# epam/Zstandard

Measured on AMD Instinct MI355X. Metric: GiB/s compress @ level 3, 64 KiB chunks, higher is better.
Workload: dtype u8; 1 GPU; 4096 independent 65536 B chunks per GPU per step, level 3, BASELINE config[1] shape (Silesia unavailable offline -> Zipf-token log stream, SURVEY 8d); chunks_per_gpu=4096, chunk_bytes=65536, level=3, parallelism=chunks sharded over 1 GPU(s), no collective in the data path

## Files before the change

zstandard_amd/csrc/lz_kernels.hip:

```cpp
#include "zsmi_device.h"
#include <type_traits>

#ifndef ZS_CAND_G
#define ZS_CAND_G 8
#endif
#ifndef ZS_CAND_G_BIG
#define ZS_CAND_G_BIG 16
#endif
#define ZS_CAND_GOF(TLOG) ((TLOG) > ZS_TABLE_LOG_SMALL ? ZS_CAND_G_BIG : ZS_CAND_G)
#ifndef ZS_CAND_DEPTH
#define ZS_CAND_DEPTH 2
#endif
#ifndef ZS_CAND_RUNS
#define ZS_CAND_RUNS 1
#endif
#define ZS_CAND_WAVES(NT) (3 * (NT))
#define ZS_CAND_ROW 65u
#define ZS_CAND_LDS(TLOG, NT) ((size_t)(NT) * (4u << (TLOG)) + 3u * (NT) * ZS_CAND_GOF(TLOG) * ZS_CAND_ROW * 4u + (NT) * 256u + 3u * 16u * 8u + 32u)
#define ZS_SLOT_EMPTY 0xFFFFFFFFu
__device__ __forceinline__ uint32_t zs_hash_short(uint32_t lo, uint32_t hi) { return __umul24(lo, 0x9E3779u) + __umul24(__builtin_amdgcn_alignbit(hi, lo, 16), 0x85EBCBu); }
__device__ __forceinline__ uint32_t zs_hash_long(uint32_t lo, uint32_t hi)
{ return __umul24(lo, 0x9E3779u) + __umul24(__builtin_amdgcn_alignbit(hi, lo, 24), 0x85EBCBu) + __umul24(hi >> 16, 0xC2B2AFu); }

template <int TLOG, int NT, bool PFX = false>
__global__ void __launch_bounds__(64 * ZS_CAND_WAVES(NT))
k_lz_candidates(const uint8_t *__restrict__ src, const ZsUnitDesc *__restrict__ units, uint32_t block0,
                uint16_t *__restrict__ distAll, uint8_t *__restrict__ distHiAll, uint32_t *__restrict__ candCount,
                const uint32_t *__restrict__ dictImg = nullptr, uint32_t pfx = 0)
{
    static_assert(!PFX || TLOG == ZS_TABLE_LOG_BIG, "a prefixed unit spans up to 128 KiB of positions");
    extern __shared__ __attribute__((aligned(16))) uint32_t candLds[];
    constexpr bool BIG = TLOG > ZS_TABLE_LOG_SMALL;
    constexpr uint32_t G = ZS_CAND_GOF(TLOG), GP = G * 64u, H = G / NT;
    constexpr uint32_t M = ZS_CAND_DEPTH;
    constexpr uint32_t LPS = 64u / G;
    constexpr uint32_t WD = G / 4u + 2u;
    static_assert(G == 8 || G == 16, "a hasher lane takes G consecutive positions of a group: 8 or 16");
    const uint32_t wave = (uint32_t)__builtin_amdgcn_readfirstlane((int)(threadIdx.x >> 6)), lane = threadIdx.x & 63u;
    const uint32_t tab = (wave < NT) ? wave : ((wave < 2 * NT) ? wave - NT : wave - 2 * NT);
    uint32_t *T = candLds + ((size_t)tab << TLOG);
    uint32_t *opnd = candLds + ((size_t)NT << TLOG);
    constexpr uint32_t ROW = ZS_CAND_ROW, GR = G * ROW;
    constexpr uint32_t RING = 3u * NT * GR;
    uint64_t *runMarks = reinterpret_cast<uint64_t *>(opnd + RING + NT * 64u);
    uint32_t *runFlag = opnd + RING + NT * 64u + 3u * 16u * 2u;
    const ZsUnitDesc ud = units[blockIdx.x];
    const uint8_t *s = src + ud.srcOff;
    const uint32_t n = ud.size;
    const size_t slot = (size_t)(ud.firstBlock - block0);
    uint16_t *dist = distAll + slot * ZS_BLOCK_MAX;
    uint8_t *distHi = distHiAll + slot * (ZS_BLOCK_MAX / 8);
    const uint32_t hashable = (n >= 8) ? n - 7 : 0;
    const uint32_t nGroups = (hashable + GP - 1) / GP;
    if (threadIdx.x < 2) candCount[2 * slot + threadIdx.x] = 0;
    if (nGroups == 0) return;
    if (n >= 16 && (n & 15u) == 0) {
        uint4 f;
        __builtin_memcpy(&f, s, 16);
        const uint32_t splat = (f.x & 0xFFu) * 0x01010101u;
        if (((f.x ^ splat) | (f.y ^ splat) | (f.z ^ splat) | (f.w ^ splat)) == 0) {
            if (threadIdx.x == 0) candLds[0] = 0;
            __syncthreads();
            uint32_t mixed = 0;
            for (uint32_t i = threadIdx.x * 16u; i < n && !mixed; i += ZS_CAND_WAVES(NT) * 64u * 16u) {
                uint4 v;
                __builtin_memcpy(&v, s + i, 16);
                mixed = (v.x ^ splat) | (v.y ^ splat) | (v.z ^ splat) | (v.w ^ splat);
            }
            if (mixed) candLds[0] = 1u;
            __syncthreads();
            const bool uniform = candLds[0] == 0;
            __syncthreads();
            if (uniform) return;
        }
    }
    const uint32_t dummyBase = ((uint32_t)(NT - tab) << TLOG) + RING + tab * 64u;
    auto mergeRead = [&](uint32_t g, uint32_t (&mS)[H], uint32_t (&mL)[H]) {
        const uint32_t *xb = opnd + (size_t)(g % 3u) * NT * GR + (NT > 1 ? tab * H : 0u) * ROW + lane;
        #pragma unroll
        for (uint32_t uu = 0; uu < H; uu++) { mS[uu] = xb[uu * ROW]; mL[uu] = (NT > 1) ? xb[GR + uu * ROW] : 0u; }
    };
    uint32_t found = 0;
    const uint32_t matchlessBelow = n >> ZS_MATCHLESS_SHIFT;
    auto mergeStore = [&](uint32_t g, const uint32_t (&mS)[H], const uint32_t (&mL)[H]) {
        const uint32_t sbase = g * GP + ((NT > 1) ? tab * H * 64u : 0u);
        uint64_t hiMine = 0;
        #pragma unroll
        for (uint32_t uu = 0; uu < H; uu++) {
            const uint32_t dm = (NT > 1) ? (mL[uu] ? mL[uu] : mS[uu]) : mS[uu];
            if (BIG) { const uint64_t hi = __ballot((dm >> 16) != 0); if (lane == uu) hiMine = hi; }
            if (found < matchlessBelow) {
                if ((g + 1u) * GP <= hashable) found += (uint32_t)__popcll(__ballot(dm != 0));
                else found += (uint32_t)__popcll(__ballot(dm != 0 && sbase + uu * 64 + lane < hashable));
            }
            dist[sbase + uu * 64 + lane] = (uint16_t)dm;
        }
        if (BIG && lane < H) *reinterpret_cast<uint64_t *>(distHi + ((sbase + lane * 64) >> 3)) = hiMine;
    };
    if (wave >= 2 * NT) {
        __syncthreads(); __syncthreads();
        for (uint32_t i = 2; i <= nGroups + 1; i++) {
            uint32_t mS[H], mL[H];
            mergeRead(i - 2, mS, mL);
#if ZS_CAND_RUNS
            if (__builtin_amdgcn_readfirstlane((int)runFlag[((i - 2) % 3u) * 2u + tab])) {
                if (lane == 0) runFlag[((i - 2) % 3u) * 2u + tab] = 0;
                #pragma unroll
                for (uint32_t uu = 0; uu < H; uu++) {
                    const uint64_t marks = runMarks[((i - 2) % 3u) * 16u + ((NT > 1) ? tab * H : 0u) + uu];
                    if ((marks >> lane) & 1ull) { if (NT > 1) mL[uu] = 1u; else mS[uu] = 1u; }
                }
            }
#endif
            mergeStore(i - 2, mS, mL);
            __syncthreads();
        }
        if (lane == 0) candCount[2 * slot + tab] = found;
        return;
    }

    if (wave < NT) {
        if constexpr (PFX) {
            uint4 *t4 = reinterpret_cast<uint4 *>(T);
            const uint4 *img4 = reinterpret_cast<const uint4 *>(dictImg + ((size_t)tab << TLOG));
            #pragma unroll 8
            for (uint32_t i = lane; i < (1u << TLOG) / 4; i += 64) t4[i] = img4[i];
        } else {
            uint4 *t4 = reinterpret_cast<uint4 *>(T);
            const uint4 e = make_uint4(ZS_SLOT_EMPTY, ZS_SLOT_EMPTY, ZS_SLOT_EMPTY, ZS_SLOT_EMPTY);
            #pragma unroll 8
            for (uint32_t i = lane; i < (1u << TLOG) / 4; i += 64) t4[i] = e;
        }
        uint32_t ringSlot = 0;
        __syncthreads();
        for (uint32_t i = 1; i <= nGroups; i++) {
            uint32_t *ob = opnd + ((size_t)ringSlot * NT + tab) * GR + lane;
            const uint32_t base = (i - 1) * GP + lane + (PFX ? pfx : 0u);
            uint32_t op[G], entry[G], old[G];
            #pragma unroll
            for (uint32_t u = 0; u < G; u++) op[u] = ob[u * ROW];
            #pragma unroll
            for (uint32_t u = 0; u < G; u++) {
                uint32_t pu = base + u * 64u;
                asm volatile("" : "+v"(pu));
                entry[u] = (op[u] & 0xFFFE0000u) | pu;
                old[u] = atomicExch(&T[op[u] & 0xFFFFu], entry[u]);
            }
            #pragma unroll
            for (uint32_t u = 0; u < G; u++) {
                const uint32_t x = old[u] ^ entry[u], dd = entry[u] - old[u];
                ob[u * ROW] = (max(x, dd) < (1u << 17)) ? dd : 0u;
            }
            ringSlot = (ringSlot == 2u) ? 0u : ringSlot + 1u;
            __syncthreads();
        }
        __syncthreads();
        return;
    }

    auto run = [&](auto roleTag) {
        constexpr bool LONG = decltype(roleTag)::value;
        const uint32_t stepOfLane = lane / LPS, l0 = (lane % LPS) * G;
        const uint32_t wbase = stepOfLane * ROW + l0;
        const uint32_t last8 = n - 8;
        auto loadGroup = [&](uint32_t g, uint32_t (&w)[WD]) {
            const uint32_t o = g * GP + lane * G;
            #pragma unroll
            for (uint32_t k = 0; k < WD / 2; k++) {
                const uint32_t ok = o + 8u * k, oc = min(ok, last8);
                const uint64_t v = zs_load64(s + oc) >> (8u * min(ok - oc, 7u));
                w[2 * k] = (uint32_t)v; w[2 * k + 1] = (uint32_t)(v >> 32);
            }
        };
        uint32_t bufA[M][WD], bufB[M][WD];
        auto loadM = [&](uint32_t g0, uint32_t (&buf)[M][WD]) {
            #pragma unroll
            for (uint32_t k = 0; k < M; k++) loadGroup(min(g0 + k, nGroups), buf[k]);
        };
        auto iter = [&](auto wholeTag, uint32_t i, const uint32_t (&w)[WD]) {
            constexpr bool WHOLE = decltype(wholeTag)::value;
            const uint32_t ringSlot = i % 3u;
            if (i < nGroups) {
                uint32_t *ob = opnd + ((size_t)ringSlot * NT + tab) * GR + wbase;
                const uint32_t pbase = i * GP + lane * G;
                #pragma unroll
                for (uint32_t u = 0; u < G; u++) {
                    const uint32_t k = u >> 2, sh = u & 3u;
                    const uint32_t lo = sh ? __builtin_amdgcn_alignbyte(w[k + 1], w[k], sh) : w[k];
                    const uint32_t hi = sh ? __builtin_amdgcn_alignbyte(w[min(k + 2, WD - 1)], w[k + 1], sh) : w[k + 1];
                    uint32_t h = LONG ? zs_hash_long(lo, hi) : zs_hash_short(lo, hi);
                    asm volatile("" : "+v"(h));
                    const uint32_t r = __builtin_amdgcn_alignbit(h, h, 32 - TLOG);
                    ob[u] = (WHOLE || pbase + u < hashable) ? (r & (0xFFFE0000u | ((1u << TLOG) - 1u))) : ((r & 0xFFFE0000u) | (dummyBase + l0 + u));
                }
#if ZS_CAND_RUNS
                bool flat = false;
                uint64_t flatLanes = 0;
                if (WHOLE && __ballot(w[0] == w[1])) {
                    uint32_t diff = w[0] ^ __builtin_amdgcn_alignbyte(w[0], w[0], 1);
                    #pragma unroll
                    for (uint32_t k = 1; k < WD; k++) diff |= w[k] ^ w[k - 1];
                    flat = diff == 0;
                    flatLanes = __ballot(flat);
                }
                if (flatLanes) {
                    const uint32_t key = flat ? ((w[0] & 0xFFu) | 0x100u) : 0u;
                    const uint32_t keyBelow = (uint32_t)__builtin_amdgcn_update_dpp(0, (int)key, 0x138, 0xF, 0xF, true);
                    const uint32_t keyAbove = (uint32_t)__builtin_amdgcn_update_dpp(0, (int)key, 0x130, 0xF, 0xF, true);
                    const bool markFirst = flat && keyBelow == key && (lane % LPS) != 0u;
                    const bool innerLast = flat && keyAbove == key && (lane % LPS) != LPS - 1u;
                    if (flat) {
                        uint32_t h = LONG ? zs_hash_long(w[0], w[1]) : zs_hash_short(w[0], w[1]);
                        asm volatile("" : "+v"(h));
                        const uint32_t away = (__builtin_amdgcn_alignbit(h, h, 32 - TLOG) & 0xFFFE0000u) | (dummyBase + l0);
                        if (markFirst) ob[0] = away;
                        #pragma unroll
                        for (uint32_t u = 1; u + 1 < G; u++) ob[u] = away + u;
                        if (innerLast) ob[G - 1] = away + (G - 1);
                    }
                    if (!LONG) {
                        if (lane < NT) runFlag[ringSlot * 2u + lane] = 1u;
                        const uint32_t bits = flat ? (((1u << G) - 2u) | (markFirst ? 1u : 0u)) : 0u;
                        if (G == 8) reinterpret_cast<uint8_t *>(runMarks + ringSlot * 16u)[lane] = (uint8_t)bits;
                        else reinterpret_cast<uint16_t *>(runMarks + ringSlot * 16u)[lane] = (uint16_t)bits;
                    }
                }
#endif
            }
            __syncthreads();
        };
        auto step = [&](uint32_t i, const uint32_t (&w)[WD]) {
            if (i > nGroups + 1) return;
            if ((i + 1) * GP + 8u <= n) iter(std::true_type{}, i, w); else iter(std::false_type{}, i, w);
        };
#if ZS_CAND_RUNS
        if (!LONG && lane < 6u) runFlag[lane] = 0;
#endif
        loadM(0, bufA);
        for (uint32_t g0 = 0; g0 <= nGroups + 1; g0 += 2 * M) {
            loadM(g0 + M, bufB);
            #pragma unroll
            for (uint32_t k = 0; k < M; k++) step(g0 + k, bufA[k]);
            loadM(g0 + 2 * M, bufA);
            #pragma unroll
            for (uint32_t k = 0; k < M; k++) step(g0 + M + k, bufB[k]);
        }
    };
    if (tab == 0) run(std::false_type{}); else run(std::true_type{});
}

__global__ void __launch_bounds__(1024)
k_lz_dict_tables(const uint8_t *__restrict__ pre, uint32_t pfx, uint32_t *__restrict__ img)
{
    constexpr int TLOG = ZS_TABLE_LOG_BIG;
    __shared__ uint32_t T[1u << TLOG];
    const uint32_t tab = blockIdx.x, tid = threadIdx.x;
    for (uint32_t i = tid; i < (1u << TLOG); i += 1024) T[i] = 0;
    __syncthreads();
    const uint32_t hashable = pfx >= 8 ? pfx - 7 : 0;
    for (uint32_t p = tid; p < hashable; p += 1024) {
        const uint64_t v = zs_load64(pre + p);
        const uint32_t lo = (uint32_t)v, hi = (uint32_t)(v >> 32);
        const uint32_t h = tab ? zs_hash_long(lo, hi) : zs_hash_short(lo, hi);
        const uint32_t r = __builtin_amdgcn_alignbit(h, h, 32 - TLOG);
        atomicMax(&T[r & ((1u << TLOG) - 1u)], ((p + 1u) << 15) | (r >> 17));
    }
    __syncthreads();
    uint32_t *out = img + ((size_t)tab << TLOG);
    for (uint32_t i = tid; i < (1u << TLOG); i += 1024) {
        const uint32_t k = T[i];
        out[i] = k ? (((k & 0x7FFFu) << 17) | ((k >> 15) - 1u)) : ZS_SLOT_EMPTY;
    }
}

#ifndef ZS_WALK_MASK
#define ZS_WALK_MASK 2
#endif
#ifndef ZS_WALK_MINW
#define ZS_WALK_MINW 1
#endif
#define ZS_WALK_WGRP(WLOG) ((WLOG) >= 9 ? 4 : 2)
#ifndef ZS_WALK_LPW_256
#define ZS_WALK_LPW_256 2
#endif
#ifndef ZS_WALK_LPW_512
#define ZS_WALK_LPW_512 4
#endif
#define ZS_WALK_LPW(WLOG) ((WLOG) >= 9 ? ZS_WALK_LPW_512 : ZS_WALK_LPW_256)
#define ZS_WALK_THREADS(BIG, WLOG) ((((BIG) ? ZS_UNIT_MAX : ZS_BLOCK_MAX) >> (WLOG)) * ZS_WALK_LPW(WLOG))
#define ZS_WALK_KERNEL(LOOK, REPW, BIG, WLOG) k_lz_walk<ZS_WALK_LPW(WLOG), ZS_WALK_WGRP(WLOG), LOOK, REPW, BIG, ZS_WALK_THREADS(BIG, WLOG)>
#ifndef ZS_WALK_SKEW
#define ZS_WALK_SKEW  24u
#endif
#define ZS_WALK_FRONT 48u
#define ZS_WALK_TAIL  144u
#define ZS_WALK_SRCBYTES(CAPB) ((((CAPB) + ZS_WALK_TAIL + ZS_WALK_SKEW * (((CAPB) + ZS_WALK_TAIL) / 256u + 1u)) + 15u) & ~15u)
#define ZS_WALK_LDS(CAPB) ((CAPB) / 8 + 16 + ZS_WALK_FRONT + ZS_WALK_SRCBYTES(CAPB) + 16 + 1024)

typedef const __attribute__((address_space(3))) uint32_t *ZsLdsU32;
template <int K>
__device__ __forceinline__ void lds_span(uint32_t byteOff, uint32_t (&out)[K])
{
    ZsLdsU32 d = (ZsLdsU32)(uintptr_t)(byteOff & ~3u);
    uint32_t w[K + 1];
    #pragma unroll
    for (int k = 0; k <= K; k++) w[k] = d[k];
    const uint32_t sh = byteOff & 3u;
    #pragma unroll
    for (int k = 0; k < K; k++) out[k] = __builtin_amdgcn_alignbyte(w[k + 1], w[k], sh);
}
template <int I, int K>
__device__ __forceinline__ uint32_t span_at(const uint32_t (&v)[K])
{
    if constexpr ((I & 3) == 0) return v[I >> 2];
    else return __builtin_amdgcn_alignbyte(v[(I >> 2) + 1], v[I >> 2], I & 3);
}
__device__ __forceinline__ uint32_t zs_agree16(const uint32_t (&a)[4], const uint32_t (&b)[4])
{
    const uint64_t x0 = (uint64_t)(a[0] ^ b[0]) | ((uint64_t)(a[1] ^ b[1]) << 32), x1 = (uint64_t)(a[2] ^ b[2]) | ((uint64_t)(a[3] ^ b[3]) << 32);
    const uint32_t n0 = x0 ? ((uint32_t)__builtin_ctzll(x0) >> 3) : 8u;
    const uint32_t n1 = x1 ? ((uint32_t)__builtin_ctzll(x1) >> 3) : 8u;
    return (n0 < 8u) ? n0 : 8u + n1;
}
template <int LPW> __device__ __forceinline__ uint32_t walker_or(uint32_t v)
{
    if constexpr (LPW >= 2) v |= (uint32_t)__builtin_amdgcn_update_dpp(0, (int)v, 0xB1, 0xF, 0xF, false);
    if constexpr (LPW == 4) v |= (uint32_t)__builtin_amdgcn_update_dpp(0, (int)v, 0x4E, 0xF, 0xF, false);
    return v;
}
template <int LPW> __device__ __forceinline__ int walker_max(int v)
{
    if constexpr (LPW >= 2) v = max(v, __builtin_amdgcn_update_dpp(0, v, 0xB1, 0xF, 0xF, false));
    if constexpr (LPW == 4) v = max(v, __builtin_amdgcn_update_dpp(0, v, 0x4E, 0xF, 0xF, false));
    return v;
}
template <int LPW> __device__ __forceinline__ uint32_t walker_min(uint32_t v)
{
    if constexpr (LPW >= 2) v = min(v, (uint32_t)__builtin_amdgcn_update_dpp(0, (int)v, 0xB1, 0xF, 0xF, false));
    if constexpr (LPW == 4) v = min(v, (uint32_t)__builtin_amdgcn_update_dpp(0, (int)v, 0x4E, 0xF, 0xF, false));
    return v;
}
template <int NT, int DIR>
__device__ __forceinline__ uint32_t block_scan_max(uint32_t v, uint32_t *wv, uint32_t tid, uint32_t *total)
{
    const uint32_t lane = tid & 63u, wave = tid >> 6;
    #pragma unroll
    for (int d = 1; d < 64; d <<= 1) {
        const uint32_t o = (uint32_t)(DIR > 0 ? __shfl_up((int)v, d) : __shfl_down((int)v, d));
        if (DIR > 0 ? (int)lane >= d : (int)lane + d < 64) v = max(v, o);
    }
    __syncthreads();
    if (lane == (DIR > 0 ? 63u : 0u)) wv[wave] = v;
    __syncthreads();
    uint32_t pre = 0, all = 0;
    #pragma unroll
    for (uint32_t k = 0; k < NT / 64; k++) { const uint32_t x = wv[k]; all = max(all, x); if (DIR > 0 ? k < wave : k > wave) pre = max(pre, x); }
    *total = all;
    return max(v, pre);
}
__device__ __forceinline__ uint32_t zs_nonzero8(const uint4 d)
{
    typedef uint16_t u16x2 __attribute__((ext_vector_type(2)));
    const u16x2 one = { 1, 1 };
    (void)one;
    auto nz = [&](uint32_t w) { uint32_t r; asm("v_pk_min_u16 %0, %1, %2" : "=v"(r) : "v"(w), "v"(0x00010001u)); return r; };
    const uint32_t v = nz(d.x) | (nz(d.y) << 2) | (nz(d.z) << 4) | (nz(d.w) << 6);
    return (v | (v >> 15)) & 0xFFu;
}

#ifdef ZS_WALK_PROFILE
#define WPROF_STAMP(k) { __builtin_amdgcn_sched_barrier(0); unsigned long long t_; asm volatile("s_waitcnt vmcnt(0) lgkmcnt(0)\n\ts_memtime %0\n\ts_waitcnt lgkmcnt(0)" : "=s"(t_) :: "memory"); __builtin_amdgcn_sched_barrier(0); wprof[k] += t_ - wlast; wlast = t_; }
#else
#define WPROF_STAMP(k)
#endif
#define ZS_WALK_KERNEL_PFX(LOOK, REPW, WLOG) k_lz_walk<ZS_WALK_LPW(WLOG), ZS_WALK_WGRP(WLOG), LOOK, REPW, true, ZS_WALK_THREADS(false, WLOG), true>
template <int LPW, int WGRP, int LOOK, int REPWIN, bool BIG, int NT, bool PFX = false>
__global__ void __launch_bounds__(NT, BIG ? 1 : ZS_WALK_MINW)
k_lz_walk(const uint8_t *__restrict__ src, const ZsUnitDesc *__restrict__ units, uint32_t block0,
          const uint16_t *__restrict__ distAll, const uint8_t *__restrict__ distHiAll,
          uint2 *__restrict__ recAll, uint32_t junkSlot, uint4 *__restrict__ resAll, int rangeLogArg, const uint32_t *__restrict__ candCount,
          const uint8_t *__restrict__ pre = nullptr, uint32_t pfx = 0)
{
    static_assert(!PFX || BIG, "a prefixed unit is staged in the 128 KiB layout");
    constexpr uint32_t CAP = BIG ? ZS_UNIT_MAX : ZS_BLOCK_MAX;
    constexpr uint32_t CPL = LOOK / LPW, RPL = REPWIN / LPW, GPL = WGRP / LPW;
    static_assert((LPW == 1 || LPW == 2 || LPW == 4) && WGRP % LPW == 0 && LOOK % LPW == 0 && REPWIN % LPW == 0 && CPL >= 1 && RPL >= 1 && LOOK <= 8 && REPWIN <= 8, "a walker's lanes share the groups and candidates evenly");
    static_assert(NT >= 64 && NT % 64 == 0 && NT * GPL * 16 <= CAP / 8, "the exchange buffer holds 16 bytes a lane and group");
    extern __shared__ __attribute__((aligned(16))) uint8_t walkLds[];
    constexpr uint32_t SRC = CAP / 8 + 16 + ZS_WALK_FRONT;
    auto lposv = [](uint32_t v) { return SRC + v + (uint32_t)__mul24((int)v >> 8, (int)ZS_WALK_SKEW); };
    const uint32_t vb = PFX ? pfx : 0u;
    auto lpos = [&](uint32_t p) { return lposv(p + vb); };
    auto stage16 = [&](uint32_t i, const uint4 v) {
        uint8_t *d = walkLds + lposv(i);
        *reinterpret_cast<uint2 *>(d) = make_uint2(v.x, v.y); *reinterpret_cast<uint2 *>(d + 8) = make_uint2(v.z, v.w);
        const uint32_t o = i & 255u;
        if (o == 0) { *reinterpret_cast<uint2 *>(d - ZS_WALK_SKEW) = make_uint2(v.x, v.y); *reinterpret_cast<uint2 *>(d - ZS_WALK_SKEW + 8) = make_uint2(v.z, v.w); }
        else if (o == 16) *reinterpret_cast<uint2 *>(d - ZS_WALK_SKEW) = make_uint2(v.x, v.y);
    };
    const uint32_t tid = threadIdx.x, lane = tid & 63u;
    const uint32_t rangeLog = (uint32_t)rangeLogArg, R = 1u << rangeLog;
    const ZsUnitDesc ud = units[blockIdx.x];
    const uint32_t slot = ud.firstBlock - block0;
    const uint8_t *s = src + ud.srcOff;
    const uint32_t n = ud.size;
    const uint16_t *dist = distAll + (size_t)slot * ZS_BLOCK_MAX;
    const uint8_t *distHi = distHiAll + (size_t)slot * (ZS_BLOCK_MAX / 8);
    uint4 *xbuf = reinterpret_cast<uint4 *>(walkLds);
    const uint32_t xw = (tid & ~63u) * GPL;
    const uint32_t safeAddr = (xw + lane) * 16u;
    uint32_t *queue = reinterpret_cast<uint32_t *>(walkLds + SRC + ZS_WALK_SRCBYTES(CAP));
    uint4 *res = resAll + (size_t)slot * ZS_RES_PER_BLOCK;
    uint8_t *xhi = reinterpret_cast<uint8_t *>(queue + 4);
    uint2 *recs = recAll + (size_t)slot * (ZS_BLOCK_MAX / 4);
    const uint32_t sub = lane & (LPW - 1u);
#ifdef ZS_WALK_PROFILE
    unsigned long long wprof[10] = { 0, 0, 0, 0, 0, 0, 0, 0, 0, 0 }, wlast;
    asm volatile("s_memtime %0\n\ts_waitcnt lgkmcnt(0)" : "=s"(wlast) :: "memory");
#endif

    if (candCount[2 * slot] + candCount[2 * slot + 1] < (n >> ZS_MATCHLESS_SHIFT)) {
        const uint32_t nRanges = (n + R - 1) >> rangeLog, perBlockLog = 16u - rangeLog;
        for (uint32_t r = tid; r < nRanges; r += NT) res[(r >> perBlockLog) * ZS_RES_PER_BLOCK + (r & ((1u << perBlockLog) - 1u))] = make_uint4(0, 0, 0, 0);
        return;
    }
    uint32_t mixed = 0;
    if (tid < (ZS_WALK_FRONT - ZS_WALK_SKEW) / 4) reinterpret_cast<uint32_t *>(walkLds + SRC - ZS_WALK_FRONT)[tid] = 0;
    if (tid == 0) { queue[0] = 0; queue[1] = 0; }
    __syncthreads();
    if constexpr (PFX) {
        const uint32_t end = pfx + n, splat = (n ? (uint32_t)s[0] : 0u) * 0x01010101u;
        for (uint32_t i = tid * 16; i < end + ZS_WALK_TAIL && i + 16 <= CAP + ZS_WALK_TAIL; i += NT * 16) {
            uint4 w = make_uint4(0, 0, 0, 0);
            if (i + 16 <= pfx) __builtin_memcpy(&w, pre + i, 16);
            else if (i >= pfx && i + 16 <= end) {
                __builtin_memcpy(&w, s + (i - pfx), 16);
                mixed |= (w.x ^ splat) | (w.y ^ splat) | (w.z ^ splat) | (w.w ^ splat);
            } else if (i < end) {
                uint8_t b[16];
                for (uint32_t k = 0; k < 16; k++) {
                    const uint32_t v = i + k;
                    b[k] = v < pfx ? pre[v] : (v < end ? s[v - pfx] : (uint8_t)0);
                    if (v >= pfx && v < end && b[k] != (uint8_t)splat) mixed = 1;
                }
                __builtin_memcpy(&w, b, 16);
            }
            stage16(i, w);
        }
        if ((n & 15u) != 0 || n < 16) mixed = 1;
    } else {
        constexpr uint32_t PER = (CAP / 16 + NT - 1) / NT;
        const uint32_t nFull = n & ~15u;
        uint4 v[PER];
        const uint32_t splat = (n ? (uint32_t)s[0] : 0u) * 0x01010101u;
        #pragma unroll
        for (uint32_t k = 0; k < PER; k++) {
            const uint32_t i = (tid + k * NT) * 16;
            const uint32_t ii = (i + 16 <= nFull) ? i : 0u;
            v[k] = make_uint4(0, 0, 0, 0);
            if (nFull >= 16) __builtin_memcpy(&v[k], s + ii, 16);
        }
        #pragma unroll
        for (uint32_t k = 0; k < PER; k++) {
            const uint32_t i = (tid + k * NT) * 16;
            if (i + 16 <= nFull) stage16(i, v[k]);
            mixed |= (v[k].x ^ splat) | (v[k].y ^ splat) | (v[k].z ^ splat) | (v[k].w ^ splat);
        }
        if (n != nFull || n < 16) mixed = 1;
        for (uint32_t i = nFull + tid * 16; i < n + ZS_WALK_TAIL; i += NT * 16) {
            uint4 w = make_uint4(0, 0, 0, 0);
            if (i < n) {
                uint64_t lo = 0, hi = 0;
                for (uint32_t k = 0; k < 16 && i + k < n; k++) { const uint64_t c = s[i + k]; if (k < 8) lo |= c << (8 * k); else hi |= c << (8 * (k - 8)); }
                w = make_uint4((uint32_t)lo, (uint32_t)(lo >> 32), (uint32_t)hi, (uint32_t)(hi >> 32));
            }
            if (i + 16 <= CAP + ZS_WALK_TAIL) stage16(i, w);
        }
    }
#if defined(ZS_WALK_STOP) && ZS_WALK_STOP == 1
    if (n) return;
#endif
    const uint32_t hashable = (n >= 8) ? n - 7 : 0;
    if (mixed) queue[1] = 1u;
    __syncthreads();
    if (queue[1] == 0) {
        const uint32_t nRanges = (n + R - 1) >> rangeLog, perBlockLog = 16u - rangeLog;
        for (uint32_t r = tid; r < nRanges; r += NT) res[(r >> perBlockLog) * ZS_RES_PER_BLOCK + (r & ((1u << perBlockLog) - 1u))] = make_uint4(0, 0, 0, 0);
        return;
    }
    WPROF_STAMP(0)

    {
        const uint32_t nRanges = (n + R - 1) >> rangeLog;
        bool active = false, more = true;
        uint32_t r = 0, ip = 0, anchor = 0, scanEnd = 0, limit = 0, rep0 = 0, rep1 = 0, nseq = 0, lastOff = 0, recBase = 0, blockBase = 0;
        uint2 heldRec = make_uint2(0, 0);
        const uint32_t perBlockLog = 16u - rangeLog;
        auto resIndex = [&](uint32_t rr) { return (rr >> perBlockLog) * ZS_RES_PER_BLOCK + (rr & ((1u << perBlockLog) - 1u)); };
        typedef __attribute__((address_space(3))) uint4 *ZsLdsU4;
        const uint32_t xwaveLds = (uint32_t)__builtin_amdgcn_readfirstlane((int)(uint32_t)(uintptr_t)(ZsLdsU4)(xbuf + xw));
        uint32_t gh[GPL] = {};
        auto loadGroup = [&](uint32_t p) {
            #pragma unroll
            for (uint32_t k = 0; k < GPL; k++) {
                const uint32_t g = (p >> 3) + sub + LPW * k;
                const uint16_t *gsrc = dist + (size_t)g * 8u;
                uint32_t keep;
                asm volatile("s_mov_b32 %0, m0\n\ts_mov_b32 m0, %2\n\ts_nop 0\n\tglobal_load_lds_dwordx4 %1, off\n\ts_mov_b32 m0, %0" : "=&s"(keep) : "v"(gsrc), "s"(xwaveLds + k * 1024u) : "memory");
                if (BIG) gh[k] = (uint32_t)distHi[g];
            }
        };
        for (;;) {
            if (__any(!active && more)) {
                const uint64_t idle = __ballot(!active && more && sub == 0);
                uint32_t base = 0;
                if (lane == 0) base = atomicAdd(queue, (uint32_t)__popcll(idle));
                base = (uint32_t)__builtin_amdgcn_readfirstlane((int)base);
                if (!active && more) {
                    const uint32_t leader = lane & ~(LPW - 1u);
                    r = base + (uint32_t)__popcll(idle & ((1ull << leader) - 1ull));
                    if (r >= nRanges) more = false;
                    else {
                        const uint32_t start = r << rangeLog;
                        const uint32_t blockStart = start & ~(ZS_BLOCK_MAX - 1);
                        const uint32_t blockEnd = blockStart + min(n - blockStart, ZS_BLOCK_MAX);
                        const uint32_t end = min(start + R, blockEnd);
                        limit = min(end + ZS_CROSS_MAX, blockEnd);
                        scanEnd = (blockEnd - blockStart >= 16) ? min(end, hashable) : 0;
                        ip = start; anchor = start; rep0 = 0; rep1 = 0; nseq = 0; lastOff = 0; recBase = start >> 2; blockBase = blockStart;
                        active = ip < scanEnd;
                        if (!active && sub == 0) res[resIndex(r)] = make_uint4(0, 0, 0, 0);
                        if (active) { loadGroup(ip); asm volatile("s_waitcnt vmcnt(0)" ::: "memory"); }
                    }
                }
            }
            if (!__any(active)) { if (!__any(more)) break; continue; }
            WPROF_STAMP(1)
#ifdef ZS_WALK_PROFILE
            wprof[8] += 1; wprof[9] += (unsigned long long)__popcll(__ballot(active));
#endif
            const uint32_t wend = min((ip & ~7u) + 8u * WGRP, scanEnd);
            uint32_t rm0 = 0, rm1 = 0;
            {
                const bool t0 = active && rep0 != 0 && ip + vb >= rep0, t1 = active && rep1 != 0 && ip + vb >= rep1;
                const uint32_t p0 = ip + sub * RPL;
                constexpr int SP = (RPL + 3 + 3) / 4;
                uint32_t a[SP] = {}, b[SP] = {}, c[SP] = {};
                if (ZS_WALK_MASK != 1 || t0 || t1) {
                    const bool tr = ZS_WALK_MASK != 2 || t0 || t1;
                    lds_span<SP>(tr ? lpos(p0) : safeAddr, a);
                    lds_span<SP>(tr ? lpos(t0 ? p0 - rep0 : p0) : safeAddr, b);
                    lds_span<SP>(tr ? lpos(t1 ? p0 - rep1 : p0) : safeAddr, c);
                }
                auto tryAt = [&](auto iTag) {
                    constexpr int I = decltype(iTag)::value;
                    const uint32_t q = p0 + I;
                    const bool ok = q < wend && q + 4 <= limit;
                    const uint32_t av = span_at<I>(a);
                    if (t0 && ok && av == span_at<I>(b)) rm0 |= 1u << (sub * RPL + I);
                    if (t1 && ok && av == span_at<I>(c)) rm1 |= 1u << (sub * RPL + I);
                };
                tryAt(std::integral_constant<int, 0>{});
                if constexpr (RPL >= 2) tryAt(std::integral_constant<int, 1>{});
                if constexpr (RPL >= 4) { tryAt(std::integral_constant<int, 2>{}); tryAt(std::integral_constant<int, 3>{}); }
                if constexpr (RPL >= 8) { tryAt(std::integral_constant<int, 4>{}); tryAt(std::integral_constant<int, 5>{}); tryAt(std::integral_constant<int, 6>{}); tryAt(std::integral_constant<int, 7>{}); }
                rm0 = walker_or<LPW>(rm0); rm1 = walker_or<LPW>(rm1);
                rm1 &= ~rm0;
            }
            WPROF_STAMP(2)
            asm volatile("s_waitcnt vmcnt(0)" ::: "memory");
            uint32_t m = 0;
            #pragma unroll
            for (uint32_t k = 0; k < GPL; k++) {
                const uint4 gd = xbuf[xw + 64u * k + lane];
                if (BIG) xhi[xw + 64u * k + lane] = (uint8_t)gh[k];
                m |= (zs_nonzero8(gd) | gh[k]) << (8u * (sub + LPW * k));
            }
            m = walker_or<LPW>(m) >> (ip & 7u);
            if (active) m = (m & (0xFFFFFFFFu >> (32u - (wend - ip)))) | rm0 | rm1; else m = 0;
            {
                const uint32_t skip = sub * CPL;
                if constexpr ((LPW - 1) * CPL >= 4) { uint32_t t = m & (m - 1); t &= t - 1; t &= t - 1; t &= t - 1; m = (skip & 4u) ? t : m; }
                if constexpr ((((LPW - 1) * CPL) & 2) != 0 || (LPW == 4 && CPL == 2)) { uint32_t t = m & (m - 1); t &= t - 1; m = (skip & 2u) ? t : m; }
                if constexpr ((CPL & 1) != 0) { const uint32_t t = m & (m - 1); m = (skip & 1u) ? t : m; }
            }
            uint32_t idx[CPL], off[CPL], dv[CPL]; bool have[CPL], isRep[CPL];
            #pragma unroll
            for (uint32_t c = 0; c < CPL; c++) {
                have[c] = m != 0;
                idx[c] = have[c] ? (uint32_t)__builtin_ctz(m) : 0u;
                m &= m - 1;
                const uint32_t q = ip + idx[c];
                const uint32_t j = (q >> 3) - (ip >> 3);
                const uint32_t owner = xw + 64u * (j / LPW) + (lane & ~(LPW - 1u)) + (j % LPW);
                dv[c] = reinterpret_cast<const uint16_t *>(xbuf + owner)[q & 7u];
                if (BIG) dv[c] |= (((uint32_t)xhi[owner] >> (q & 7u)) & 1u) << 16;
            }
            #pragma unroll
            for (uint32_t c = 0; c < CPL; c++) asm volatile("" : "+v"(dv[c]));
            #pragma unroll
            for (uint32_t c = 0; c < CPL; c++) {
                const bool r0 = ((rm0 >> idx[c]) & 1u) != 0, r1 = ((rm1 >> idx[c]) & 1u) != 0;
                isRep[c] = have[c] && (r0 || r1);
                off[c] = r0 ? rep0 : (r1 ? rep1 : dv[c]);
                if (!have[c]) off[c] = 0;
            }
            WPROF_STAMP(3)
            int bestKey = 0; uint32_t bestPack = 0, bestOff = 0;
            uint32_t sa[CPL][3], sb[CPL][3];
            #pragma unroll
            for (uint32_t c = 0; c < CPL; c++) {
                const uint32_t q = ip + idx[c];
                #pragma unroll
                for (int k = 0; k < 3; k++) { sa[c][k] = 0; sb[c][k] = 0; }
                if (ZS_WALK_MASK != 1 || have[c]) {
                    const bool tr = ZS_WALK_MASK != 2 || have[c];
                    lds_span<3>(tr ? lpos(q - 4) : safeAddr, sa[c]);
                    lds_span<3>(tr ? lpos(q - off[c] - 4) : safeAddr, sb[c]);
                }
            }
            if (ZS_WALK_MASK != 1) {
                #pragma unroll
                for (uint32_t c = 0; c < CPL; c++) asm volatile("" : "+v"(sa[c][0]), "+v"(sa[c][1]), "+v"(sa[c][2]), "+v"(sb[c][0]), "+v"(sb[c][1]), "+v"(sb[c][2]));
            }
            #pragma unroll
            for (uint32_t c = 0; c < CPL; c++) {
                const uint32_t q = ip + idx[c];
                const uint32_t (&a)[3] = sa[c], (&b)[3] = sb[c];
                const uint32_t xb = a[0] ^ b[0], x0 = a[1] ^ b[1], x1 = a[2] ^ b[2];
                const uint32_t f0 = x0 ? (uint32_t)__builtin_ctz(x0) : 32u, f1 = x1 ? (uint32_t)__builtin_ctz(x1) : 32u;
                const uint32_t fwd = min(((x0 ? f0 : 32u + f1)) >> 3, limit - q);
                const uint32_t maxBack = min(min(q - anchor, q + vb - off[c]), ZS_BCAP);
                const uint32_t back = min(xb ? ((uint32_t)__builtin_clz(xb) >> 3) : 4u, maxBack);
                if (have[c] && fwd >= (isRep[c] ? ZS_REPMIN : ZS_MINMATCH)) {
                    const int gain = (int)(4u * fwd + 8u * back) - (isRep[c] ? 0 : (int)zs_highbit(off[c] + 1)) - 5 * (int)idx[c];
                    const int key = ((gain + 2048) << 3) | (int)(7u - (sub * CPL + c));
                    if (key > bestKey) { bestKey = key; bestPack = idx[c] | (fwd << 8) | (back << 16); bestOff = off[c]; }
                }
            }
            const int best = walker_max<LPW>(bestKey);
            const bool took = active && best != 0;
            const uint32_t packed = walker_or<LPW>(bestKey == best ? bestPack : 0u), boff = walker_or<LPW>(bestKey == best ? bestOff : 0u);
            const uint32_t bq = ip + (packed & 0xFFu), bback = packed >> 16;
            uint32_t bfwd = (packed >> 8) & 0xFFu;
            WPROF_STAMP(4)
            const bool extend = took && bfwd == ZS_FCAP && (limit - bq) > ZS_FCAP;
            bool need = extend;
            uint32_t pos = bq + ZS_FCAP;
            while (__any(need)) {
                uint32_t e = 0xFFFFFFFFu;
                if (need) {
                    const uint32_t cap = limit - pos, fo = 16u * sub;
                    uint32_t nb = 0;
                    if (fo < cap) {
                        uint32_t a[4], b[4];
                        lds_span<4>(lpos(pos + fo), a);
                        lds_span<4>(lpos(pos - boff + fo), b);
                        nb = zs_agree16(a, b);
                    }
                    if (nb < 16u || fo + 16u >= cap) e = min(fo + nb, cap);
                }
                e = walker_min<LPW>(e);
                if (need) {
                    if (e != 0xFFFFFFFFu) { pos += e; need = false; }
                    else pos += 16u * LPW;
                }
            }
            if (extend) bfwd = pos - bq;
            WPROF_STAMP(5)
            uint32_t recLl = 0;
            if (took) {
                recLl = bq - bback - anchor;
                nseq++; lastOff = boff;
                ip = bq + bfwd; anchor = ip;
                if (boff == rep1) { rep1 = rep0; rep0 = boff; }
                else if (boff != rep0) { rep1 = rep0; rep0 = boff; }
            } else if (active) ip = wend;
            if (took) {
                const uint2 rec = make_uint2((bq - bback - blockBase) | ((bback + bfwd) << 17), boff | (recLl << 17));
                if (nseq & 1u) heldRec = rec;
                else if (sub == 0) *reinterpret_cast<uint4 *>(recs + recBase + nseq - 2) = make_uint4(heldRec.x, heldRec.y, rec.x, rec.y);
            }
            if (active && ip >= scanEnd) {
                if (sub == 0) {
                    if (nseq & 1u) recs[recBase + nseq - 1] = heldRec;
                    res[resIndex(r)] = make_uint4(nseq, nseq ? anchor - blockBase : 0u, lastOff, 0u);
                }
                active = false;
            }
            if (active) loadGroup(ip);
            WPROF_STAMP(6)
        }
    }
    WPROF_STAMP(1)
#ifdef ZS_WALK_PROFILE
    __syncthreads();
    if (lane == 0) { unsigned long long *o = reinterpret_cast<unsigned long long *>(resAll + (size_t)(junkSlot / 64)) + ((size_t)blockIdx.x * (NT / 64) + (tid >> 6)) * 10;    for (int k = 0; k < 10; k++) o[k] = wprof[k]; }
#endif
}

__global__ void __launch_bounds__(256)
k_lz_stitch(const ZsBlockDesc *__restrict__ blocks, const uint2 *__restrict__ recAll, const uint4 *__restrict__ resAll,
            ZsSeqRec *__restrict__ seqAll, ZsRangeHdr *__restrict__ hdrAll, int rangeLogArg)
{
    constexpr int NT = 256;
    __shared__ uint32_t sa[9 * 256 + 16];
    uint32_t *sKept = sa, *sCnt = sa + 256, *sTrail = sa + 512, *sFOut = sa + 768, *sNs = sa + 1024, *sOwn = sa + 1280, *sEs = sa + 1536, *sPend = sa + 1792, *sChain = sa + 2048, *sWave = sa + 2304;
    const uint32_t tid = threadIdx.x, lane = tid & 63u;
    const uint32_t rangeLog = (uint32_t)rangeLogArg, R = 1u << rangeLog;
    const uint32_t slot = blockIdx.x;
    const uint32_t NRB = ZS_BLOCK_MAX >> rangeLog;
    const uint32_t gLog = ZS_OUT_LOG - rangeLog, G = 1u << gLog;
    const uint2 *recs = recAll + (size_t)slot * (ZS_BLOCK_MAX / 4);
    const uint4 *res = resAll + (size_t)slot * ZS_RES_PER_BLOCK;
    {
        const uint32_t bStart = 0, bi = 0;
        const uint32_t bN = blocks[slot].size;
        const uint32_t bEnd = bN;
        const uint32_t t = tid;
        const bool mine = t < NRB;
        const bool walked = mine && bN >= 16 && (t << rangeLog) < bN;
        const uint4 rr = walked ? res[t] : make_uint4(0, 0, 0, 0);
        const uint32_t ns = rr.x, le = rr.y;
        const uint32_t rs = min(bStart + (t << rangeLog), bEnd), re = min(bStart + (t << rangeLog) + R, bEnd);
        const uint2 *rp = recs + ((bStart + (t << rangeLog)) >> 2);
        uint32_t total;
        const uint32_t key = ns ? ((le << 9) | (511u - t)) : 0u;
        const uint32_t incl = block_scan_max<NT, 1>(key, sWave, tid, &total);
        uint32_t excl = (uint32_t)__shfl_up((int)incl, 1);
        if (lane == 0) { excl = 0; for (uint32_t k = 0; k < (tid >> 6); k++) excl = max(excl, sWave[k]); }
        const uint32_t own = max(excl >> 9, bStart), reach = max(incl >> 9, bStart), reachAll = max(total >> 9, bStart);
        const uint32_t definer = 511u - (excl & 511u);
#if defined(ZS_STITCH_STOP) && ZS_STITCH_STOP == 2
        if (bN) return;
#endif
        uint32_t f = 0, fStart = 0, fEnd = 0, fOff = 0;
        if (ns && own >= rs) {
            if (le <= own) f = ns;
            else {
                const uint4 r01 = *reinterpret_cast<const uint4 *>(rp);
                auto endOf = [](uint32_t x) { return (x & 0x1FFFFu) + (x >> 17); };
                uint2 rec = make_uint2(r01.x, r01.y), nxt = make_uint2(r01.z, r01.w);
                bool haveNxt = ns > 1;
                if (endOf(r01.x) > own) f = 0;
                else if (ns > 1 && endOf(r01.z) > own) { f = 1; rec = nxt; haveNxt = false; }
                else {
                    uint32_t lo = 2, hi = ns - 1;
                    while (lo < hi) { const uint32_t mid = (lo + hi) >> 1; if (endOf(rp[mid].x) > own) hi = mid; else lo = mid + 1; }
                    f = lo; rec = rp[f]; haveNxt = false;
                }
                uint32_t st = rec.x & 0x1FFFFu, en = endOf(rec.x);
                if (st < own && en - own < ZS_MINMATCH) {
                    f++;
                    if (f < ns) { rec = haveNxt ? nxt : rp[f]; st = rec.x & 0x1FFFFu; en = endOf(rec.x); }
                }
                fStart = max(st, own); fEnd = en; fOff = rec.y & 0x1FFFFu;
            }
        }
        const bool keptAny = f < ns;
        if (mine) sKept[t] = keptAny;
        __syncthreads();
        const bool joined = keptAny && excl != 0 && own >= rs && fStart == own && fOff == res[definer].z && sKept[definer] != 0;
        const uint32_t fOut = f + (joined ? 1u : 0u), cnt = ns - fOut;
        const uint32_t es = joined ? fEnd : max(rs, own), te = max(re, reach), lastEnd = cnt ? le : es;
        const bool stopper = ns && le > own && !(joined && cnt == 0);
        uint32_t total2;
        const uint32_t key2 = stopper ? (((512u - t) << 18) | (joined ? fEnd : own)) : 0u;
        const uint32_t sfx = block_scan_max<NT, -1>(key2, sWave, tid, &total2);
        uint32_t sfxEx = (uint32_t)__shfl_down((int)sfx, 1);
        if (lane == 63) { sfxEx = 0; for (uint32_t k = (tid >> 6) + 1; k < NT / 64; k++) sfxEx = max(sfxEx, sWave[k]); }
        const uint32_t chainEnd = sfxEx ? (sfxEx & 0x3FFFFu) : reachAll;
        if (mine) { sCnt[t] = cnt; sTrail[t] = te - lastEnd; sFOut[t] = fOut; sNs[t] = ns; sOwn[t] = own; sEs[t] = es; sChain[t] = chainEnd; }
        __syncthreads();
        const uint32_t gi = t & (G - 1u);
        if (mine) {
            uint32_t pend = 0;
            for (uint32_t i = gi; i > 0; i--) { pend += sTrail[t - gi + i - 1]; if (sCnt[t - gi + i - 1]) break; }
            sPend[t] = pend;
        }
        __syncthreads();
#if defined(ZS_STITCH_STOP) && ZS_STITCH_STOP == 1
        if (bN) return;
#endif
        const uint32_t wave = tid >> 6;
        for (uint32_t go = 0; go < ZS_WALK_RANGES / (NT / 64); go++) {
            const uint32_t g = wave * (ZS_WALK_RANGES / (NT / 64)) + go, j0 = g << gLog;
            uint32_t c[4] = { 0, 0, 0, 0 }, total = 0;
            for (uint32_t i = 0; i < G; i++) { c[i] = sCnt[j0 + i]; total += c[i]; }
            ZsSeqRec *out = seqAll + ((size_t)slot * ZS_WALK_RANGES + g) * ZS_SEQ_PER_RANGE;
            uint32_t lits = 0;
            for (uint32_t d0 = 0; d0 < total; d0 += 64) {
                const uint32_t d = d0 + lane;
                if (d < total) {
                    uint32_t j = 0, pre = 0;
                    if (d >= c[0]) { j = 1; pre = c[0]; if (G > 2) { if (d >= pre + c[1]) { j = 2; pre += c[1]; if (d >= pre + c[2]) { j = 3; pre += c[2]; } } } }
                    const uint32_t jr = j0 + j, k = sFOut[jr] + (d - pre);
                    const uint2 rec = recs[(jr << (rangeLog - 2)) + k];
                    uint32_t st = rec.x & 0x1FFFFu, ml = rec.x >> 17, ll = rec.y >> 17;
                    const uint32_t off = rec.y & 0x1FFFFu, en = st + ml;
                    if (d == pre) {
                        const uint32_t ownj = sOwn[jr];
                        if (st < ownj) { st = ownj; ml = en - st; }
                        ll = st - sEs[jr] + sPend[jr];
                    }
                    if (k + 1 == sNs[jr]) ml = sChain[jr] - st;
                    ZsSeqRec w; w.x = zs_rec_x(ll, ml, off); w.y = zs_rec_y(off, st);
                    out[d] = w;
                    lits += ll;
                }
            }
            #pragma unroll
            for (int o = 32; o >= 1; o >>= 1) lits += (uint32_t)__shfl_xor((int)lits, o);
            if (lane == 0) {
                ZsRangeHdr h; h.nseq = total; h.litSum = lits; h.trailing = 0; h.first = 0;
                for (uint32_t i = G; i > 0; i--) { h.trailing += sTrail[j0 + i - 1]; if (sCnt[j0 + i - 1]) break; }
                hdrAll[(size_t)slot * ZS_WALK_RANGES + g] = h;
            }
        }
    }
}
```

Measured before the change: 140.9 GiB/s.

## Replace atomic range queue in LZ walk with static assignment and optional lane parking

Drops the per-wave atomic work queue that handed out ranges in the LZ walk kernel. Each lane group now gets exactly one range from its thread index. An optional second phase, enabled by ZS_WALK_PARK_AT, parks still-active walker state in LDS once a wave falls below a lane threshold, then repacks it densely across waves for a compaction pass. The goal is to cut atomic and scheduling overhead. With the default of 0 parking is off, so this relies on there being at most one range per lane group; if a block holds more ranges than lane groups, some would go unprocessed.

```diff
diff --git a/zstandard_amd/csrc/lz_kernels.hip b/zstandard_amd/csrc/lz_kernels.hip
--- a/zstandard_amd/csrc/lz_kernels.hip
+++ b/zstandard_amd/csrc/lz_kernels.hip
@@ -295,7 +295,7 @@
 #define ZS_WALK_FRONT 48u
 #define ZS_WALK_TAIL  144u
 #define ZS_WALK_SRCBYTES(CAPB) ((((CAPB) + ZS_WALK_TAIL + ZS_WALK_SKEW * (((CAPB) + ZS_WALK_TAIL) / 256u + 1u)) + 15u) & ~15u)
-#define ZS_WALK_LDS(CAPB) ((CAPB) / 8 + 16 + ZS_WALK_FRONT + ZS_WALK_SRCBYTES(CAPB) + 16 + 1024)
+#define ZS_WALK_LDS(CAPB) ((CAPB) / 8 + 16 + ZS_WALK_FRONT + ZS_WALK_SRCBYTES(CAPB) + 16 + 1024 + 64)
 
 typedef const __attribute__((address_space(3))) uint32_t *ZsLdsU32;
 template <int K>
@@ -412,6 +412,7 @@
     uint32_t *queue = reinterpret_cast<uint32_t *>(walkLds + SRC + ZS_WALK_SRCBYTES(CAP));
     uint4 *res = resAll + (size_t)slot * ZS_RES_PER_BLOCK;
     uint8_t *xhi = reinterpret_cast<uint8_t *>(queue + 4);
+    uint32_t *parkedOf = reinterpret_cast<uint32_t *>(xhi + 1024);
     uint2 *recs = recAll + (size_t)slot * (ZS_BLOCK_MAX / 4);
     const uint32_t sub = lane & (LPW - 1u);
 #ifdef ZS_WALK_PROFILE
@@ -426,7 +427,7 @@
     }
     uint32_t mixed = 0;
     if (tid < (ZS_WALK_FRONT - ZS_WALK_SKEW) / 4) reinterpret_cast<uint32_t *>(walkLds + SRC - ZS_WALK_FRONT)[tid] = 0;
-    if (tid == 0) { queue[0] = 0; queue[1] = 0; }
+    if (tid == 0) queue[1] = 0;
     __syncthreads();
     if constexpr (PFX) {
         const uint32_t end = pfx + n, splat = (n ? (uint32_t)s[0] : 0u) * 0x01010101u;
@@ -492,11 +493,26 @@
 
     {
         const uint32_t nRanges = (n + R - 1) >> rangeLog;
-        bool active = false, more = true;
-        uint32_t r = 0, ip = 0, anchor = 0, scanEnd = 0, limit = 0, rep0 = 0, rep1 = 0, nseq = 0, lastOff = 0, recBase = 0, blockBase = 0;
+        constexpr uint32_t WPW = 64u / LPW;
+#ifndef ZS_WALK_PARK_AT
+#define ZS_WALK_PARK_AT 0
+#endif
+        constexpr uint32_t PARK_LANES = ZS_WALK_PARK_AT ? 64u / ZS_WALK_PARK_AT : 0u;
+        bool active = false;
+        uint32_t r = tid / LPW, ip = 0, anchor = 0, scanEnd = 0, limit = 0, rep0 = 0, rep1 = 0, nseq = 0, lastOff = 0, recBase = 0, blockBase = 0;
         uint2 heldRec = make_uint2(0, 0);
         const uint32_t perBlockLog = 16u - rangeLog;
         auto resIndex = [&](uint32_t rr) { return (rr >> perBlockLog) * ZS_RES_PER_BLOCK + (rr & ((1u << perBlockLog) - 1u)); };
+        auto rangeOf = [&](uint32_t rr) {
+            const uint32_t start = rr << rangeLog;
+            const uint32_t blockStart = start & ~(ZS_BLOCK_MAX - 1);
+            const uint32_t blockEnd = blockStart + min(n - blockStart, ZS_BLOCK_MAX);
+            const uint32_t end = min(start + R, blockEnd);
+            limit = min(end + ZS_CROSS_MAX, blockEnd);
+            scanEnd = (blockEnd - blockStart >= 16) ? min(end, hashable) : 0;
+            recBase = start >> 2; blockBase = blockStart;
+            return start;
+        };
         typedef __attribute__((address_space(3))) uint4 *ZsLdsU4;
         const uint32_t xwaveLds = (uint32_t)__builtin_amdgcn_readfirstlane((int)(uint32_t)(uintptr_t)(ZsLdsU4)(xbuf + xw));
         uint32_t gh[GPL] = {};
@@ -510,31 +526,15 @@
                 if (BIG) gh[k] = (uint32_t)distHi[g];
             }
         };
-        for (;;) {
-            if (__any(!active && more)) {
-                const uint64_t idle = __ballot(!active && more && sub == 0);
-                uint32_t base = 0;
-                if (lane == 0) base = atomicAdd(queue, (uint32_t)__popcll(idle));
-                base = (uint32_t)__builtin_amdgcn_readfirstlane((int)base);
-                if (!active && more) {
-                    const uint32_t leader = lane & ~(LPW - 1u);
-                    r = base + (uint32_t)__popcll(idle & ((1ull << leader) - 1ull));
-                    if (r >= nRanges) more = false;
-                    else {
-                        const uint32_t start = r << rangeLog;
-                        const uint32_t blockStart = start & ~(ZS_BLOCK_MAX - 1);
-                        const uint32_t blockEnd = blockStart + min(n - blockStart, ZS_BLOCK_MAX);
-                        const uint32_t end = min(start + R, blockEnd);
-                        limit = min(end + ZS_CROSS_MAX, blockEnd);
-                        scanEnd = (blockEnd - blockStart >= 16) ? min(end, hashable) : 0;
-                        ip = start; anchor = start; rep0 = 0; rep1 = 0; nseq = 0; lastOff = 0; recBase = start >> 2; blockBase = blockStart;
-                        active = ip < scanEnd;
-                        if (!active && sub == 0) res[resIndex(r)] = make_uint4(0, 0, 0, 0);
-                        if (active) { loadGroup(ip); asm volatile("s_waitcnt vmcnt(0)" ::: "memory"); }
-                    }
-                }
-            }
-            if (!__any(active)) { if (!__any(more)) break; continue; }
+        if (r < nRanges) {
+            ip = anchor = rangeOf(r);
+            active = ip < scanEnd;
+            if (!active && sub == 0) res[resIndex(r)] = make_uint4(0, 0, 0, 0);
+            if (active) loadGroup(ip);
+        }
+        for (uint32_t phase = 0;; phase++) {
+          for (;;) {
+            if ((uint32_t)__popcll(__ballot(active)) <= (phase == 0 ? PARK_LANES : 0u)) break;
             WPROF_STAMP(1)
 #ifdef ZS_WALK_PROFILE
             wprof[8] += 1; wprof[9] += (unsigned long long)__popcll(__ballot(active));
@@ -690,6 +690,37 @@
             }
             if (active) loadGroup(ip);
             WPROF_STAMP(6)
+          }
+            if (phase == 1 || PARK_LANES == 0) break;
+            asm volatile("s_waitcnt vmcnt(0)" ::: "memory");
+            {
+                const uint64_t leaders = __ballot(active && sub == 0);
+                if (active && sub == 0) {
+                    uint4 *p = xbuf + xw + 2u * (uint32_t)__popcll(leaders & ((1ull << lane) - 1ull));
+                    p[0] = make_uint4(r | (nseq << 16), ip | ((ip - anchor) << 20), rep0, rep1);
+                    p[1] = make_uint4(lastOff, heldRec.x, heldRec.y, 0u);
+                }
+                if (lane == 0) parkedOf[tid >> 6] = (uint32_t)__popcll(leaders);
+            }
+            __syncthreads();
+            const uint32_t mine = (tid >> 6) * WPW + lane / LPW;
+            uint32_t from = 0, first = 0, total = 0;
+            #pragma unroll
+            for (uint32_t k = 0; k < NT / 64; k++) {
+                total += parkedOf[k];
+                if (mine >= total) { from = k + 1; first = total; }
+            }
+            if (total == 0) break;
+            active = mine < total;
+            uint4 s0 = make_uint4(0, 0, 0, 0), s1 = s0;
+            if (active) { const uint4 *p = xbuf + from * 64u * GPL + 2u * (mine - first); s0 = p[0]; s1 = p[1]; }
+            __syncthreads();
+            if (active) {
+                r = s0.x & 0xFFFFu; nseq = s0.x >> 16; ip = s0.y & 0xFFFFFu; anchor = ip - (s0.y >> 20); rep0 = s0.z; rep1 = s0.w;
+                lastOff = s1.x; heldRec = make_uint2(s1.y, s1.z);
+                (void)rangeOf(r);
+                loadGroup(ip);
+            }
         }
     }
     WPROF_STAMP(1)
```

Result: no change. 142.2 GiB/s, median of 4 (+0.9%).
